# hugofloresgarcia/vampnet

Hardware: NVIDIA H100
Metric: codec tokens/sec (coarse 12 steps + c2f 24 steps generate, T=768, 44.1 kHz) (higher is better)
Workload: dtype bf16

## Files before the change

### vampnet_b200/csrc/api.cu

```cuda
#include <cuda_bf16.h>
#include <cudaTypedefs.h>

#include <cmath>
#include <cstdarg>
#include <cstdio>
#include <cstring>
#include <map>
#include <memory>
#include <string>
#include <tuple>
#include <vector>

#include "kernels.h"

namespace vnb {

static thread_local std::string g_err;
static thread_local std::string g_tmap_err;

static int fail(const char* fmt, ...) {
  char buf[1024];
  va_list ap;
  va_start(ap, fmt);
  vsnprintf(buf, sizeof(buf), fmt, ap);
  va_end(ap);
  g_err = buf;
  return 1;
}
#define CK(expr)                                                                                   \
  do {                                                                                             \
    cudaError_t _e = (expr);                                                                       \
    if (_e != cudaSuccess) return fail("%s failed: %s (%s:%d)", #expr, cudaGetErrorString(_e), __FILE__, __LINE__); \
  } while (0)

static PFN_cuTensorMapEncodeTiled_v12000 get_encode() {
  static PFN_cuTensorMapEncodeTiled_v12000 fn = nullptr;
  if (fn) return fn;
  void* p = nullptr;
  cudaDriverEntryPointQueryResult q;
  cudaError_t e = cudaGetDriverEntryPoint("cuTensorMapEncodeTiled", &p, cudaEnableDefault, &q);
  if (e != cudaSuccess || q != cudaDriverEntryPointSuccess || !p) {
    g_tmap_err = std::string("cudaGetDriverEntryPoint(cuTensorMapEncodeTiled) failed: ") + cudaGetErrorString(e);
    return nullptr;
  }
  fn = reinterpret_cast<PFN_cuTensorMapEncodeTiled_v12000>(p);
  return fn;
}
const char* tmap_error() { return g_tmap_err.c_str(); }

bool make_tmap_2d(CUtensorMap* tm, const void* base, uint64_t rows, uint64_t cols, uint32_t box_rows,
                  uint32_t box_cols) {
  auto enc = get_encode();
  if (!enc) return false;
  cuuint64_t dims[2] = {cols, rows};
  cuuint64_t strides[1] = {cols * 2};
  cuuint32_t box[2] = {box_cols, box_rows};
  cuuint32_t estr[2] = {1, 1};
  CUresult r = enc(tm, CU_TENSOR_MAP_DATA_TYPE_BFLOAT16, 2, const_cast<void*>(base), dims, strides, box, estr,
                   CU_TENSOR_MAP_INTERLEAVE_NONE, CU_TENSOR_MAP_SWIZZLE_128B, CU_TENSOR_MAP_L2_PROMOTION_L2_256B,
                   CU_TENSOR_MAP_FLOAT_OOB_FILL_NONE);
  if (r != CUDA_SUCCESS) {
    char b[256];
    snprintf(b, sizeof(b), "cuTensorMapEncodeTiled(2d rows=%llu cols=%llu box=%ux%u) -> %d", (unsigned long long)rows,
             (unsigned long long)cols, box_rows, box_cols, (int)r);
    g_tmap_err = b;
    return false;
  }
  return true;
}
bool make_tmap_3d(CUtensorMap* tm, const void* base, uint64_t batch, uint64_t rows, uint64_t cols,
                  uint64_t pitch_elems, uint32_t box_rows, uint32_t box_cols) {
  auto enc = get_encode();
  if (!enc) return false;
  cuuint64_t dims[3] = {cols, rows, batch};
  cuuint64_t strides[2] = {pitch_elems * 2, rows * pitch_elems * 2};
  cuuint32_t box[3] = {box_cols, box_rows, 1};
  cuuint32_t estr[3] = {1, 1, 1};
  CUresult r = enc(tm, CU_TENSOR_MAP_DATA_TYPE_BFLOAT16, 3, const_cast<void*>(base), dims, strides, box, estr,
                   CU_TENSOR_MAP_INTERLEAVE_NONE, CU_TENSOR_MAP_SWIZZLE_128B, CU_TENSOR_MAP_L2_PROMOTION_L2_256B,
                   CU_TENSOR_MAP_FLOAT_OOB_FILL_NONE);
  if (r != CUDA_SUCCESS) {
    char b[256];
    snprintf(b, sizeof(b), "cuTensorMapEncodeTiled(3d batch=%llu rows=%llu cols=%llu pitch=%llu box=%ux%u) -> %d",
             (unsigned long long)batch, (unsigned long long)rows, (unsigned long long)cols,
             (unsigned long long)pitch_elems, box_rows, box_cols, (int)r);
    g_tmap_err = b;
    return false;
  }
  return true;
}

static bool make_gemm_plan(GemmPlan* p, int epi, const void* A, const void* W, int M, int N, int K, void* out,
                           void* out2, const float* bias, int T, int Tpad, const float* ss_in, int ss_parts,
                           float inv_d, float eps, void* out_bf16, float* ss_out) {
  if (N % 256 != 0 || K % 64 != 0 || M < 1) {
    g_tmap_err = "gemm: need N % 256 == 0 and K % 64 == 0";
    return false;
  }
  GemmArgs& a = p->args;
  a.M = M; a.N = N; a.K = K; a.epi = epi; a.out = out; a.out2 = out2; a.bias = bias;
  a.T = T; a.Tpad = Tpad; a.d2 = epi == VNB_EPI_QKV ? (N / 3) * 2 : 0;
  if (ss_in != nullptr) { a.ss_in = ss_in; a.ss_parts = ss_parts; a.inv_d = inv_d; a.eps = eps; }
  a.out_bf16 = reinterpret_cast<__nv_bfloat16*>(out_bf16); a.ss_out = ss_out;
  return make_tmap_2d(&p->tmA, A, M, K, 128, 64) && make_tmap_2d(&p->tmB, W, N, K, 256, 64) &&
         make_tmap_2d(&p->tmBh, W, N, K, 128, 64);
}

bool make_attn_plan(AttnPlan* p, const void* qk, const void* vT, void* out, const float* rel, int sat, int B, int T,
                    int Tpad, int H) {
  const int d = H * 64;
  p->out = out; p->rel = rel; p->sat = sat; p->B = B; p->T = T; p->Tpad = Tpad; p->H = H;
  return make_tmap_3d(&p->tmQ, qk, B, T, 2 * d, 2 * d, 128, 64) && make_tmap_3d(&p->tmK, qk, B, T, 2 * d, 2 * d, 64, 64) &&
         make_tmap_3d(&p->tmVT, vT, B, d, Tpad, Tpad, 64, 64);
}

struct DevBuf {
  void* p = nullptr;
  size_t n = 0;
  ~DevBuf() { if (p) cudaFree(p); }
  cudaError_t alloc(size_t bytes, bool zero = false) {
    n = bytes;
    cudaError_t e = cudaMalloc(&p, bytes ? bytes : 1);
    if (e == cudaSuccess && zero) e = cudaMemset(p, 0, bytes);
    return e;
  }
  template <class T> T* as() const { return reinterpret_cast<T*>(p); }
};

struct Variant {
  int steps = 0;
  bool has_mask = false;
  bool top_p = false;
  int gemm_pair = 0;
  bool fused = false;
  bool adapted = false;
  bool ragged = false;
  bool mixed_steps = false;
  bool split = false;
  bool operator<(const Variant& o) const {
    return std::tie(steps, has_mask, top_p, gemm_pair, fused, adapted, ragged, mixed_steps, split) <
           std::tie(o.steps, o.has_mask, o.top_p, o.gemm_pair, o.fused, o.adapted, o.ragged, o.mixed_steps, o.split);
  }
};

struct Workspace {
  int B = 0, T = 0, Tpad = 0, M = 0;
  unsigned long long last_use = 0;
  DevBuf x, y, qk, vT, att, h, logits, zcur, zorig, tokens, conf, n0, dyn, rowgrp, z_in, mask_in, z_out, ssA, ssB, embA,
      partials;
  DevBuf grp_adapter, lora_u;
  DevBuf frames;
  DevBuf live;
  int embKp = 0;
  int ss_parts = 0;
  std::vector<GemmPlan> qkv, wo, up, down;
  GemmPlan cls, emb;
  GemmPlan cls_sample;
  bool can_fuse = false;
  AttnPlan attn;
  std::map<Variant, cudaGraphExec_t> graphs;
  std::map<Variant, unsigned long long> graph_kernels;
  ~Workspace() { for (auto& kv : graphs) cudaGraphExecDestroy(kv.second); }
};

}

namespace vnb {
enum { FAM_EMBED = 0, FAM_RMSNORM, FAM_GEMM_QKV, FAM_ATTN, FAM_GEMM_O, FAM_GEMM_UP, FAM_GEMM_DOWN, FAM_GEMM_CLS,
       FAM_SAMPLE, FAM_STATE, FAM_LORA_DOWN, FAM_COUNT };
static unsigned long long g_captures = 0;
static unsigned long long g_launches = 0;
void count_launch(unsigned long long n) { g_launches += n; }
struct Profiler {
  bool on = false;
  std::vector<cudaEvent_t> pool;
  std::vector<int> fam;
  size_t used = 0;
  ~Profiler() { for (auto e : pool) cudaEventDestroy(e); }
  void mark(int family, cudaStream_t st) {
    if (!on) return;
    if (used == pool.size()) {
      cudaEvent_t e;
      if (cudaEventCreate(&e) != cudaSuccess) { on = false; return; }
      pool.push_back(e);
      fam.push_back(-1);
    }
    fam[used] = family;
    cudaEventRecord(pool[used++], st);
// ... 1180 lines not shown
```

### vampnet_b200/csrc/common.cuh

```cuda
#pragma once
#include <cuda.h>
#include <cuda_bf16.h>
#include <cuda_runtime.h>
#include <stdint.h>
#include <stdio.h>

namespace vnb {

__device__ __forceinline__ uint32_t smem_u32(const void* p) {
  return static_cast<uint32_t>(__cvta_generic_to_shared(p));
}
__device__ __forceinline__ uint32_t lane_id() { return threadIdx.x & 31; }

__device__ __forceinline__ bool elect_one() {
  uint32_t pred = 0;
  asm volatile(
      "{\n\t.reg .pred P;\n\t.reg .b32 R;\n\t"
      "elect.sync R|P, 0xffffffff;\n\t"
      "selp.u32 %0, 1, 0, P;\n\t}"
      : "=r"(pred));
  return pred != 0;
}

__device__ __forceinline__ void mbar_init(uint64_t* bar, uint32_t count) {
  asm volatile("mbarrier.init.shared::cta.b64 [%0], %1;" ::"r"(smem_u32(bar)), "r"(count) : "memory");
}
__device__ __forceinline__ void mbar_fence_init() {
  asm volatile("fence.mbarrier_init.release.cluster;" ::: "memory");
}
__device__ __forceinline__ void mbar_expect_tx(uint64_t* bar, uint32_t bytes) {
  asm volatile("mbarrier.arrive.expect_tx.shared::cta.b64 _, [%0], %1;" ::"r"(smem_u32(bar)), "r"(bytes)
               : "memory");
}
__device__ __forceinline__ void mbar_arrive(uint64_t* bar) {
  asm volatile("mbarrier.arrive.shared::cta.b64 _, [%0];" ::"r"(smem_u32(bar)) : "memory");
}
__device__ __forceinline__ bool mbar_try_wait(uint64_t* bar, uint32_t parity) {
  uint32_t ok;
  asm volatile(
      "{\n\t.reg .pred P;\n\t"
      "mbarrier.try_wait.parity.shared::cta.b64 P, [%1], %2, %3;\n\t"
      "selp.u32 %0, 1, 0, P;\n\t}"
      : "=r"(ok)
      : "r"(smem_u32(bar)), "r"(parity), "r"(100000u)
      : "memory");
  return ok != 0;
}
__device__ __forceinline__ uint64_t global_timer_ns() {
  uint64_t t;
  asm volatile("mov.u64 %0, %%globaltimer;" : "=l"(t));
  return t;
}
#ifndef VNB_WAIT_TIMEOUT_NS
#define VNB_WAIT_TIMEOUT_NS 4000000000ull
#endif
__device__ __forceinline__ void mbar_wait(uint64_t* bar, uint32_t parity) {
  if (mbar_try_wait(bar, parity)) return;
  const uint64_t t0 = global_timer_ns();
  while (!mbar_try_wait(bar, parity))
    if (global_timer_ns() - t0 > VNB_WAIT_TIMEOUT_NS) __trap();
}

__device__ __forceinline__ void mbar_init_a(uint32_t bar, uint32_t count) {
  asm volatile("mbarrier.init.shared::cta.b64 [%0], %1;" ::"r"(bar), "r"(count) : "memory");
}
__device__ __forceinline__ void mbar_expect_tx_a(uint32_t bar, uint32_t bytes) {
  asm volatile("mbarrier.arrive.expect_tx.shared::cta.b64 _, [%0], %1;" ::"r"(bar), "r"(bytes) : "memory");
}
__device__ __forceinline__ void mbar_arrive_a(uint32_t bar) {
  asm volatile("mbarrier.arrive.shared::cta.b64 _, [%0];" ::"r"(bar) : "memory");
}
__device__ __forceinline__ bool mbar_try_wait_a(uint32_t bar, uint32_t parity) {
  uint32_t ok;
  asm volatile(
      "{\n\t.reg .pred P;\n\t"
      "mbarrier.try_wait.parity.shared::cta.b64 P, [%1], %2, %3;\n\t"
      "selp.u32 %0, 1, 0, P;\n\t}"
      : "=r"(ok)
      : "r"(bar), "r"(parity), "r"(100000u)
      : "memory");
  return ok != 0;
}
__device__ __forceinline__ void mbar_wait_a(uint32_t bar, uint32_t parity) {
  if (mbar_try_wait_a(bar, parity)) return;
  const uint64_t t0 = global_timer_ns();
  while (!mbar_try_wait_a(bar, parity))
    if (global_timer_ns() - t0 > VNB_WAIT_TIMEOUT_NS) __trap();
}

__device__ __forceinline__ void fence_proxy_async_smem() {
  asm volatile("fence.proxy.async.shared::cta;" ::: "memory");
}

__device__ __forceinline__ void tma_prefetch_desc(const CUtensorMap* m) {
  asm volatile("prefetch.tensormap [%0];" ::"l"(reinterpret_cast<uint64_t>(m)) : "memory");
}
__device__ __forceinline__ void tma_load_2d(void* dst, const CUtensorMap* m, uint64_t* bar, int c0, int c1) {
  asm volatile(
      "cp.async.bulk.tensor.2d.shared::cluster.global.mbarrier::complete_tx::bytes [%0], [%1, {%3, %4}], [%2];"
      ::"r"(smem_u32(dst)), "l"(reinterpret_cast<uint64_t>(m)), "r"(smem_u32(bar)), "r"(c0), "r"(c1)
      : "memory");
}
__device__ __forceinline__ void tma_load_3d(void* dst, const CUtensorMap* m, uint64_t* bar, int c0, int c1, int c2) {
  asm volatile(
      "cp.async.bulk.tensor.3d.shared::cluster.global.mbarrier::complete_tx::bytes [%0], [%1, {%3, %4, %5}], [%2];"
      ::"r"(smem_u32(dst)), "l"(reinterpret_cast<uint64_t>(m)), "r"(smem_u32(bar)), "r"(c0), "r"(c1), "r"(c2)
      : "memory");
}

__device__ __forceinline__ void tma_load_3d_a(uint32_t dst, const CUtensorMap* m, uint32_t bar, int c0, int c1, int c2) {
  asm volatile(
      "cp.async.bulk.tensor.3d.shared::cluster.global.mbarrier::complete_tx::bytes [%0], [%1, {%3, %4, %5}], [%2];"
      ::"r"(dst), "l"(reinterpret_cast<uint64_t>(m)), "r"(bar), "r"(c0), "r"(c1), "r"(c2)
      : "memory");
}

__device__ __forceinline__ void tma_store_2d(const CUtensorMap* m, const void* src, int c0, int c1) {
  asm volatile("cp.async.bulk.tensor.2d.global.shared::cta.bulk_group [%0, {%2, %3}], [%1];"
               ::"l"(reinterpret_cast<uint64_t>(m)), "r"(smem_u32(src)), "r"(c0), "r"(c1)
               : "memory");
}
__device__ __forceinline__ void bulk_commit() { asm volatile("cp.async.bulk.commit_group;" ::: "memory"); }
template <int N>
__device__ __forceinline__ void bulk_wait_read() {
  asm volatile("cp.async.bulk.wait_group.read %0;" ::"n"(N) : "memory");
}

__device__ __forceinline__ uint32_t cluster_ctarank() {
  uint32_t r;
  asm volatile("mov.u32 %0, %%cluster_ctarank;" : "=r"(r));
  return r;
}
__device__ __forceinline__ void cluster_sync_all() {
  asm volatile("barrier.cluster.arrive.release.aligned;\n\tbarrier.cluster.wait.acquire.aligned;" ::: "memory");
}
__device__ __forceinline__ uint32_t mapa_u32(uint32_t cta_addr, uint32_t rank) {
  uint32_t r;
  asm volatile("mapa.shared::cluster.u32 %0, %1, %2;" : "=r"(r) : "r"(cta_addr), "r"(rank));
  return r;
}
__device__ __forceinline__ void mbar_arrive_cluster(uint32_t cluster_addr) {
  asm volatile("mbarrier.arrive.release.cluster.shared::cluster.b64 _, [%0];" ::"r"(cluster_addr) : "memory");
}
__device__ __forceinline__ bool mbar_try_wait_cluster(uint64_t* bar, uint32_t parity) {
  uint32_t ok;
  asm volatile(
      "{\n\t.reg .pred P;\n\t"
      "mbarrier.try_wait.parity.acquire.cluster.shared::cta.b64 P, [%1], %2, %3;\n\t"
      "selp.u32 %0, 1, 0, P;\n\t}"
      : "=r"(ok)
      : "r"(smem_u32(bar)), "r"(parity), "r"(100000u)
      : "memory");
  return ok != 0;
}
__device__ __forceinline__ void mbar_wait_cluster(uint64_t* bar, uint32_t parity) {
  if (mbar_try_wait_cluster(bar, parity)) return;
  const uint64_t t0 = global_timer_ns();
  while (!mbar_try_wait_cluster(bar, parity))
    if (global_timer_ns() - t0 > VNB_WAIT_TIMEOUT_NS) __trap();
}
__device__ __forceinline__ void tma_load_2d_mc(void* dst, const CUtensorMap* m, uint64_t* bar, int c0, int c1,
                                               uint16_t cta_mask) {
  asm volatile(
      "cp.async.bulk.tensor.2d.shared::cluster.global.mbarrier::complete_tx::bytes.multicast::cluster"
      " [%0], [%1, {%3, %4}], [%2], %5;"
      ::"r"(smem_u32(dst)), "l"(reinterpret_cast<uint64_t>(m)), "r"(smem_u32(bar)), "r"(c0), "r"(c1), "h"(cta_mask)
      : "memory");
}

__device__ __forceinline__ uint32_t pack_bf16x2(float lo, float hi) {
  __nv_bfloat162 v = __floats2bfloat162_rn(lo, hi);
  return *reinterpret_cast<uint32_t*>(&v);
}
__device__ __forceinline__ float fast_exp2(float x) {
  float y;
  asm volatile("ex2.approx.ftz.f32 %0, %1;" : "=f"(y) : "f"(x));
  return y;
}
__device__ __forceinline__ float lds_f32(uint32_t addr) {
  float v;
  asm volatile("ld.shared.f32 %0, [%1];" : "=f"(v) : "r"(addr));
  return v;
}
__device__ __forceinline__ void sts_f32(uint32_t addr, float v) {
  asm volatile("st.shared.f32 [%0], %1;" ::"r"(addr), "f"(v) : "memory");
}
__device__ __forceinline__ void sts_u32(uint32_t addr, uint32_t v) {
  asm volatile("st.shared.b32 [%0], %1;" ::"r"(addr), "r"(v) : "memory");
}
__device__ __forceinline__ float4 lds_f4(uint32_t addr) {
  float4 v;
  asm volatile("ld.shared.v4.f32 {%0, %1, %2, %3}, [%4];" : "=f"(v.x), "=f"(v.y), "=f"(v.z), "=f"(v.w) : "r"(addr));
  return v;
}
__device__ __forceinline__ uint2 lds_u2(uint32_t addr) {
  uint2 v;
  asm volatile("ld.shared.v2.b32 {%0, %1}, [%2];" : "=r"(v.x), "=r"(v.y) : "r"(addr));
  return v;
}
__device__ __forceinline__ void sts_f4(uint32_t addr, float4 v) {
  asm volatile("st.shared.v4.f32 [%0], {%1, %2, %3, %4};" ::"r"(addr), "f"(v.x), "f"(v.y), "f"(v.z), "f"(v.w)
               : "memory");
}
__device__ __forceinline__ void sts_v4(uint32_t addr, uint32_t a, uint32_t b, uint32_t c, uint32_t d) {
  asm volatile("st.shared.v4.b32 [%0], {%1, %2, %3, %4};" ::"r"(addr), "r"(a), "r"(b), "r"(c), "r"(d) : "memory");
}
__device__ __forceinline__ float warp_max(float v) {
#pragma unroll
  for (int o = 16; o > 0; o >>= 1) v = fmaxf(v, __shfl_xor_sync(0xffffffffu, v, o));
  return v;
}
__device__ __forceinline__ float warp_sum(float v) {
#pragma unroll
  for (int o = 16; o > 0; o >>= 1) v += __shfl_xor_sync(0xffffffffu, v, o);
  return v;
}

__device__ __forceinline__ void philox4x32_10(uint32_t c0, uint32_t c1, uint32_t c2, uint32_t c3, uint32_t k0,
                                              uint32_t k1, uint32_t (&out)[4]) {
#pragma unroll
  for (int r = 0; r < 10; ++r) {
    const uint32_t hi0 = __umulhi(0xD2511F53u, c0), lo0 = 0xD2511F53u * c0;
    const uint32_t hi1 = __umulhi(0xCD9E8D57u, c2), lo1 = 0xCD9E8D57u * c2;
    const uint32_t n0 = hi1 ^ c1 ^ k0, n2 = hi0 ^ c3 ^ k1;
    c0 = n0; c1 = lo1; c2 = n2; c3 = lo0;
    k0 += 0x9E3779B9u;
    k1 += 0xBB67AE85u;
  }
  out[0] = c0; out[1] = c1; out[2] = c2; out[3] = c3;
}
__device__ __forceinline__ float u01(uint32_t x) { return (static_cast<float>(x >> 9) + 0.5f) * 1.1920928955078125e-07f; }

}
```

### vampnet_b200/csrc/gemm_wgmma.cu

```cuda
#include <stdlib.h>

#include "common.cuh"
#include "kernels.h"
#include "wgmma.cuh"

#ifndef VNB_GEMM_PAIR_DEFAULT
#define VNB_GEMM_PAIR_DEFAULT false
#endif

namespace vnb {

constexpr int BM = 128, BN = 256, BK = 64, STAGES = 4;
constexpr int A_BYTES = BM * BK * 2;
constexpr int B_BYTES = BN * BK * 2;
constexpr int STAGE_BYTES = A_BYTES + B_BYTES;
constexpr int SBIAS_BYTES = BN * 4;
constexpr int RING_BYTES = STAGES * STAGE_BYTES;
constexpr int ACC_PITCH = BN + 1;
static_assert(BM * ACC_PITCH * 4 <= RING_BYTES, "the accumulator tile overlays the ring");
static_assert(BM * ACC_PITCH * 4 + 4 * BM + 16 + 32 * BM <= RING_BYTES, "the adapted epilogue's row table follows it");
constexpr int GEMM_SMEM = RING_BYTES + SBIAS_BYTES + 1024  + 256 ;
static_assert(GEMM_SMEM <= 227 * 1024, "H100: at most 227 KiB of shared memory per block");
constexpr int GEMM_THREADS = 256 + 32;
template <int EPI> constexpr int gemm_epi_warps() { return (EPI == VNB_EPI_RESID || EPI == VNB_EPI_SAMPLE) ? 8 : 4; }
// ... 83 lines not shown
    const float rsr = __shfl_sync(0xffffffffu, rs, r);
    const uint32_t sp = quad + 4u * (r * ACC_PITCH + tc + c8);
    float x[8];
#pragma unroll
    for (int k = 0; k < 8; ++k) {
      x[k] = lds_f32(sp + 4u * k) * rsr;
      if constexpr (GEGLU) x[k] = x[k] * gelu_tanh(lds_f32(sp + 4u * (128 + k)) * rsr);
    }
    const int row = row_base + r;
    if (row < M) {
      uint4 w;
      w.x = pack_bf16x2(x[0], x[1]);
      w.y = pack_bf16x2(x[2], x[3]);
      w.z = pack_bf16x2(x[4], x[5]);
      w.w = pack_bf16x2(x[6], x[7]);
      *reinterpret_cast<uint4*>(out + static_cast<size_t>(row) * pitch + oc + c8) = w;
    }
  }
}

__device__ __forceinline__ void acc_ld_x32(uint32_t addr, uint32_t (&v)[32]) {
#pragma unroll
  for (int j = 0; j < 32; ++j) v[j] = __float_as_uint(lds_f32(addr + 4u * j));
}

template <int EPI>
__device__ __forceinline__ void lora_update(const GemmArgs& g, uint8_t* scratch, uint32_t acc_tile, int m0, int n0) {
  int uoff = 0, brow0 = n0;
  if constexpr (EPI == VNB_EPI_QKV) {
    const int d = g.N / 3;
    if (n0 >= d && n0 < 2 * d) return;
    if (n0 >= 2 * d) { uoff = 8; brow0 = n0 - d; }
  }
  const AdapterRefs& L = g.lora;
  const int t = static_cast<int>(threadIdx.x);
  int32_t* sid = reinterpret_cast<int32_t*>(scratch);
  uint32_t* smask = reinterpret_cast<uint32_t*>(scratch + 4 * BM);
  float4* su = reinterpret_cast<float4*>(scratch + 4 * BM + 16);
  constexpr int R = EPI == VNB_EPI_QKV ? 16 : 8;
  if (t < BM) {
    const int m = m0 + t;
    const int id = m < g.M ? L.grp_adapter[L.rowgrp[m / L.rows_per_grp].group] : -1;
    sid[t] = id;
    if (id >= 0) {
      su[2 * t] = __ldg(reinterpret_cast<const float4*>(L.u + static_cast<size_t>(m) * R + uoff));
      su[2 * t + 1] = __ldg(reinterpret_cast<const float4*>(L.u + static_cast<size_t>(m) * R + uoff + 4));
    }
    uint32_t bits = 0;
    for (int a = 0; a < VNB_MAX_ADAPTERS; ++a) bits |= __ballot_sync(0xffffffffu, id == a) ? (1u << a) : 0u;
    if ((t & 31) == 0) smask[t >> 5] = bits;
  }
  asm volatile("bar.sync 1, 256;" ::: "memory");
  const uint32_t present = smask[0] | smask[1] | smask[2] | smask[3];
  const int nb = EPI == VNB_EPI_QKV ? 2 * (g.N / 3) : g.N;
  const int c0 = t & 63, rq = t >> 6;
  for (int a = 0; a < VNB_MAX_ADAPTERS; ++a) {
    if (!((present >> a) & 1u)) continue;
    const float* bp = L.table[a].b[L.slot] + (static_cast<size_t>(L.layer) * nb + brow0 + c0) * 8;
    float4 b0[4], b1[4];
#pragma unroll
    for (int j = 0; j < 4; ++j) {
      b0[j] = __ldg(reinterpret_cast<const float4*>(bp + 64 * 8 * j));
      b1[j] = __ldg(reinterpret_cast<const float4*>(bp + 64 * 8 * j + 4));
    }
#pragma unroll 4
    for (int i = 0; i < BM / 4; ++i) {
      const int r = rq + 4 * i;
      if (sid[r] != a) continue;
      const float4 ua = su[2 * r], ub = su[2 * r + 1];
      const uint32_t row_addr = acc_tile + 4u * (r * ACC_PITCH + c0);
#pragma unroll
      for (int j = 0; j < 4; ++j) {
        float s = __fmul_rn(ua.x, b0[j].x);
        s = __fmaf_rn(ua.y, b0[j].y, s); s = __fmaf_rn(ua.z, b0[j].z, s); s = __fmaf_rn(ua.w, b0[j].w, s);
        s = __fmaf_rn(ub.x, b1[j].x, s); s = __fmaf_rn(ub.y, b1[j].y, s); s = __fmaf_rn(ub.z, b1[j].z, s);
        s = __fmaf_rn(ub.w, b1[j].w, s);
        const uint32_t addr = row_addr + 4u * (64 * j);
        sts_f32(addr, __fadd_rn(lds_f32(addr), s));
      }
    }
  }
}

template <int NS, typename Release>
__device__ __forceinline__ void gemm_mainloop(float (&acc)[128], uint8_t* ring, uint64_t* full_bar, int num_kb, int wg,
                                              int& stage, uint32_t& phase, Release&& release) {
#pragma unroll
  for (int i = 0; i < 128; ++i) acc[i] = 0.f;
  for (int kb = 0; kb < num_kb; ++kb) {
    mbar_wait(&full_bar[stage], phase);
    const uint32_t sa = smem_u32(ring + stage * STAGE_BYTES) + wg * (64 * 128);
    const uint32_t sb = smem_u32(ring + stage * STAGE_BYTES + A_BYTES);
    wgmma_fence();
#pragma unroll
    for (int k = 0; k < BK / 16; ++k)
      wgmma_ss_n256(acc, wgmma_desc_sw128(sa + k * 32), wgmma_desc_sw128(sb + k * 32), 1u);
    wgmma_commit();
    wgmma_wait<1>();
    wgmma_fence_regs(acc);
    if (kb > 0) release(stage == 0 ? NS - 1 : stage - 1);
    if (++stage == NS) { stage = 0; phase ^= 1; }
  }
  wgmma_wait<0>();
  wgmma_fence_regs(acc);
  if (num_kb > 0) release(stage == 0 ? NS - 1 : stage - 1);
}

template <int EPI, bool PAIR, bool ADAPT = false, bool SPLIT = false>
__global__ void __launch_bounds__(GEMM_THREADS, 1)
gemm_wgmma_kernel(const __grid_constant__ CUtensorMap tmA, const __grid_constant__ CUtensorMap tmB,
                  const GemmArgs g) {
  extern __shared__ uint8_t smem_raw[];
  uint8_t* smem = reinterpret_cast<uint8_t*>((reinterpret_cast<uintptr_t>(smem_raw) + 1023) & ~uintptr_t(1023));
  float* sbias_all = reinterpret_cast<float*>(smem + RING_BYTES);
  uint64_t* full_bar = reinterpret_cast<uint64_t*>(smem + RING_BYTES + SBIAS_BYTES);
  uint64_t* empty_bar = full_bar + STAGES;

  const int warp = threadIdx.x >> 5;
  const int lane = threadIdx.x & 31;
  const uint32_t rank = PAIR ? cluster_ctarank() : 0u;
  const int tile = PAIR ? static_cast<int>(blockIdx.x >> 1) : static_cast<int>(blockIdx.x);
  constexpr int TM = PAIR ? 2 * BM : BM;
  const int num_n = g.N / BN;
  const int num_kb = g.K / BK;
  const int m0 = (tile / num_n) * TM + static_cast<int>(rank) * BM;
  const int n0 = (tile % num_n) * BN;
  if (g.live != nullptr && (tile / num_n) * TM >= live_rows(g)) return;

  if (warp == 8 && lane == 0) {
    tma_prefetch_desc(&tmA);
    tma_prefetch_desc(&tmB);
    for (int s = 0; s < STAGES; ++s) {
      mbar_init(&full_bar[s], 1);
      mbar_init(&empty_bar[s], 8 * (PAIR ? 2 : 1));
    }
    mbar_fence_init();
  }
  if constexpr (PAIR) cluster_sync_all();
  else __syncthreads();

  if (warp == 8) {
    if (lane == 0) {
      int stage = 0;
      uint32_t phase = 0;
      for (int kb = 0; kb < num_kb; ++kb) {
        if constexpr (PAIR) mbar_wait_cluster(&empty_bar[stage], phase ^ 1);
        else mbar_wait(&empty_bar[stage], phase ^ 1);
        uint8_t* sa = smem + stage * STAGE_BYTES;
        uint8_t* sb = sa + A_BYTES;
        mbar_expect_tx(&full_bar[stage], STAGE_BYTES);
        tma_load_2d(sa, &tmA, &full_bar[stage], kb * BK, m0);
        if constexpr (PAIR)
          tma_load_2d_mc(sb + rank * (B_BYTES / 2), &tmB, &full_bar[stage], kb * BK, n0 + static_cast<int>(rank) * (BN / 2),
                         uint16_t(3));
        else
          tma_load_2d(sb, &tmB, &full_bar[stage], kb * BK, n0);
        if (++stage == STAGES) { stage = 0; phase ^= 1; }
      }
    }
    __syncwarp();
  } else {
    const int wg = warp >> 2;
    {
      float acc[128];
      const uint32_t peer_empty = PAIR ? mapa_u32(smem_u32(empty_bar), rank ^ 1u) : 0u;
      int stage = 0;
      uint32_t phase = 0;
      gemm_mainloop<STAGES>(acc, smem, full_bar, num_kb, wg, stage, phase, [&](int s) {
        if (lane == 0) {
          mbar_arrive(&empty_bar[s]);
          if constexpr (PAIR) mbar_arrive_cluster(peer_empty + 8u * s);
        }
      });
      asm volatile("bar.sync 1, 256;" ::: "memory");
      const uint32_t acc_tile = smem_u32(smem);
      const int r = wg * 64 + (warp & 3) * 16 + (lane >> 2);
      const uint32_t p0 = acc_tile + 4u * (r * ACC_PITCH + 2 * (lane & 3));
#pragma unroll
      for (int i = 0; i < 32; ++i) {
        sts_f32(p0 + 32u * i, acc[4 * i]);
        sts_f32(p0 + 32u * i + 4, acc[4 * i + 1]);
        sts_f32(p0 + 4u * (8 * ACC_PITCH) + 32u * i, acc[4 * i + 2]);
        sts_f32(p0 + 4u * (8 * ACC_PITCH) + 32u * i + 4, acc[4 * i + 3]);
      }
      asm volatile("bar.sync 1, 256;" ::: "memory");
// ... 302 lines not shown
#pragma unroll
          for (int h = 0; h < 2; ++h) {
            const float rsr = h ? rs1 : rs0;
            const uint32_t own = pack_bf16x2(acc[4 * i + 2 * h] * rsr, acc[4 * i + 2 * h + 1] * rsr);
            const uint32_t peer = __shfl_xor_sync(0xffffffffu, own, 4);
            sts_u32(stage_tile + stage_off<256>(c, (r + 8 * h) >> 1),
                    odd ? __byte_perm(peer, own, 0x7632) : __byte_perm(own, peer, 0x5410));
          }
        }
      }
      mbar_arrive(out_full);
    }
  } else {
    const int e = warp - 8;
    __nv_bfloat16* const out = reinterpret_cast<__nv_bfloat16*>(g.out);
    const int pitch = EPI == VNB_EPI_GEGLU ? g.N / 2 : g.d2;
    auto row_scales = [&](int tile) {
      if (tile < tiles) {
        const int m0 = (tile / num_n) * BM;
        for (int j = e * 32 + lane; j < BM; j += 32 * PERS_EPI_WARPS) srs[j] = row_scale(g, m0 + j);
      }
      mbar_arrive(out_free);
    };
    row_scales(blockIdx.x);
    uint32_t it = 0;
    for (int tile = blockIdx.x; tile < tiles; tile += gridDim.x, ++it) {
      const int m0 = (tile / num_n) * BM, n0 = (tile % num_n) * BN;
      mbar_wait(out_full, it & 1u);
      if constexpr (EPI == VNB_EPI_GEGLU) {
#pragma unroll 4
        for (int u = e; u < BM / 2; u += PERS_EPI_WARPS) {
          const int rr = 2 * u + (lane >> 4);
          const float4 v = lds_f4(stage_tile + stage_off<256>(rr, 4 * (lane & 15)));
          if (m0 + rr < g.M)
            *reinterpret_cast<float4*>(out + static_cast<size_t>(m0 + rr) * pitch + (n0 >> 1) + 8 * (lane & 15)) = v;
        }
      } else if (n0 < g.d2) {
#pragma unroll 4
        for (int rr = e; rr < BM; rr += PERS_EPI_WARPS) {
          const float4 v = lds_f4(stage_tile + stage_off<512>(rr, 4 * lane));
          if (m0 + rr < g.M)
            *reinterpret_cast<float4*>(out + static_cast<size_t>(m0 + rr) * pitch + n0 + 8 * lane) = v;
        }
      } else {
        const int d = g.N - g.d2;
        uint16_t* const vt = reinterpret_cast<uint16_t*>(g.out2) + static_cast<size_t>(n0 - g.d2) * g.Tpad;
        size_t off[4];
        bool ok[4];
        int bk[4];
        uint32_t keep[2] = {0xffffffffu, 0xffffffffu};
#pragma unroll
        for (int k = 0; k < 4; ++k) {
          const int m = m0 + 4 * lane + k;
          bk[k] = m / g.T;
          const int t = m - bk[k] * g.T;
          ok[k] = m < g.M;
          off[k] = static_cast<size_t>(bk[k]) * d * g.Tpad + t;
          if (ok[k] && g.frames != nullptr && t >= __ldg(g.frames + bk[k])) keep[k >> 1] &= (k & 1) ? 0xffffu : 0xffff0000u;
        }
        const bool wide = ok[3] && bk[3] == bk[0] && (off[0] & 3) == 0 && (g.Tpad & 3) == 0 &&
                          (reinterpret_cast<uintptr_t>(g.out2) & 7) == 0;
#pragma unroll 2
        for (int c = e; c < BN; c += PERS_EPI_WARPS) {
          uint2 v = lds_u2(stage_tile + stage_off<256>(c, 2 * lane));
          v.x &= keep[0];
          v.y &= keep[1];
          uint16_t* const o = vt + static_cast<size_t>(c) * g.Tpad;
          if (wide) {
            *reinterpret_cast<uint2*>(o + off[0]) = v;
          } else {
#pragma unroll
            for (int k = 0; k < 4; ++k) {
              const uint32_t w = k < 2 ? v.x : v.y;
              if (ok[k]) o[off[k]] = static_cast<uint16_t>((k & 1) ? (w >> 16) : w);
            }
          }
        }
      }
      row_scales(tile + gridDim.x);
    }
  }
}

static int g_gemm_pair = -1;
void set_gemm_pair(int on) { g_gemm_pair = on ? 1 : 0; }
static bool gemm_pair_enabled() {
  if (g_gemm_pair < 0) {
    const char* e = getenv("VNB_GEMM_PAIR");
    g_gemm_pair = e != nullptr ? (e[0] == '1') : (VNB_GEMM_PAIR_DEFAULT ? 1 : 0);
  }
  return g_gemm_pair == 1;
}
int get_gemm_pair() { return gemm_pair_enabled() ? 1 : 0; }

static int g_max_clusters[6][64];
template <int EPI>
static cudaError_t init_epi() {
  static PerDeviceOnce once;
  int dev;
  if (!once.need(&dev)) return cudaSuccess;
  cudaError_t e = cudaFuncSetAttribute(gemm_wgmma_kernel<EPI, false>, cudaFuncAttributeMaxDynamicSharedMemorySize, GEMM_SMEM);
  if (e != cudaSuccess) return e;
  e = cudaFuncSetAttribute(gemm_wgmma_kernel<EPI, true>, cudaFuncAttributeMaxDynamicSharedMemorySize, GEMM_SMEM);
  if (e != cudaSuccess) return e;
  if constexpr (EPI == VNB_EPI_QKV || EPI == VNB_EPI_RESID || EPI == VNB_EPI_GEGLU) {
    e = cudaFuncSetAttribute(gemm_wgmma_kernel<EPI, false, true>, cudaFuncAttributeMaxDynamicSharedMemorySize, GEMM_SMEM);
    if (e != cudaSuccess) return e;
    e = cudaFuncSetAttribute(gemm_wgmma_kernel<EPI, true, true>, cudaFuncAttributeMaxDynamicSharedMemorySize, GEMM_SMEM);
    if (e != cudaSuccess) return e;
  }
  if constexpr (EPI == VNB_EPI_GEGLU || EPI == VNB_EPI_QKV) {
    e = cudaFuncSetAttribute(gemm_persistent_kernel<EPI>, cudaFuncAttributeMaxDynamicSharedMemorySize, pers_smem<EPI>());
    if (e != cudaSuccess) return e;
  }
  if constexpr (EPI == VNB_EPI_SAMPLE) {
    e = cudaFuncSetAttribute(gemm_wgmma_kernel<EPI, false, false, true>, cudaFuncAttributeMaxDynamicSharedMemorySize,
                             GEMM_SMEM);
    if (e != cudaSuccess) return e;
    e = cudaFuncSetAttribute(gemm_wgmma_kernel<EPI, true, false, true>, cudaFuncAttributeMaxDynamicSharedMemorySize,
                             GEMM_SMEM);
    if (e != cudaSuccess) return e;
  }
  cudaLaunchConfig_t q = {};
  q.gridDim = dim3(2 * device_sm_count());
  q.blockDim = dim3(GEMM_THREADS);
  q.dynamicSmemBytes = GEMM_SMEM;
  cudaLaunchAttribute qa[1];
  qa[0].id = cudaLaunchAttributeClusterDimension;
  qa[0].val.clusterDim.x = 2; qa[0].val.clusterDim.y = 1; qa[0].val.clusterDim.z = 1;
  q.attrs = qa; q.numAttrs = 1;
  int n = 0;
  e = cudaOccupancyMaxActiveClusters(&n, gemm_wgmma_kernel<EPI, true>, &q);
  if (e != cudaSuccess || n <= 0) { (void)cudaGetLastError(); n = device_sm_count() / 2; }
  if (dev >= 0 && dev < 64) g_max_clusters[EPI][dev] = n;
  once.mark(dev);
  return cudaSuccess;
}
cudaError_t prepare_gemm() {
  cudaError_t e;
  if ((e = init_epi<VNB_EPI_BF16>()) != cudaSuccess) return e;
  if ((e = init_epi<VNB_EPI_QKV>()) != cudaSuccess) return e;
  if ((e = init_epi<VNB_EPI_RESID>()) != cudaSuccess) return e;
  if ((e = init_epi<VNB_EPI_GEGLU>()) != cudaSuccess) return e;
  if ((e = init_epi<VNB_EPI_BIAS_F32>()) != cudaSuccess) return e;
  return init_epi<VNB_EPI_SAMPLE>();
}

int get_gemm_max_clusters() {
  int dev = 0;
  cudaGetDevice(&dev);
  if (prepare_gemm() != cudaSuccess || dev < 0 || dev >= 64) return 0;
  return g_max_clusters[VNB_EPI_RESID][dev];
}

template <int EPI, bool ADAPT = false, bool SPLIT = false>
static cudaError_t launch_epi(const GemmPlan& p, const GemmArgs& g, cudaStream_t st) {
  cudaError_t e = init_epi<EPI>();
  if (e != cudaSuccess) return e;
  if (gemm_pair_enabled()) {
    const int clusters = ((g.M + 2 * BM - 1) / (2 * BM)) * (g.N / BN);
    cudaLaunchConfig_t cfg = {};
    cfg.gridDim = dim3(2 * clusters);
    cfg.blockDim = dim3(GEMM_THREADS);
    cfg.dynamicSmemBytes = GEMM_SMEM;
    cfg.stream = st;
    cudaLaunchAttribute attr[1];
    attr[0].id = cudaLaunchAttributeClusterDimension;
    attr[0].val.clusterDim.x = 2; attr[0].val.clusterDim.y = 1; attr[0].val.clusterDim.z = 1;
    cfg.attrs = attr; cfg.numAttrs = 1;
    return cudaLaunchKernelEx(&cfg, gemm_wgmma_kernel<EPI, true, ADAPT, SPLIT>, p.tmA, p.tmBh, g);
  }
  const int tiles = ((g.M + BM - 1) / BM) * (g.N / BN);
  if constexpr ((EPI == VNB_EPI_GEGLU || EPI == VNB_EPI_QKV) && !ADAPT) {
    const int grid = tiles < device_sm_count() ? tiles : device_sm_count();
    gemm_persistent_kernel<EPI><<<grid, PERS_THREADS, pers_smem<EPI>(), st>>>(p.tmA, p.tmB, g);
    return cudaGetLastError();
  }
  gemm_wgmma_kernel<EPI, false, ADAPT, SPLIT><<<tiles, GEMM_THREADS, GEMM_SMEM, st>>>(p.tmA, p.tmB, g);
  return cudaGetLastError();
}

cudaError_t launch_gemm(const GemmPlan& p, cudaStream_t st) {
  GemmArgs g = p.args;
  if (g.epi != VNB_EPI_QKV) g.frames = nullptr;
  if (g.lora.table != nullptr) {
    if (!g.lora.grp_adapter || !g.lora.rowgrp || !g.lora.u || g.lora.rows_per_grp < 1) return cudaErrorInvalidValue;
    switch (g.epi) {
      case VNB_EPI_QKV: return launch_epi<VNB_EPI_QKV, true>(p, g, st);
      case VNB_EPI_RESID: return launch_epi<VNB_EPI_RESID, true>(p, g, st);
      case VNB_EPI_GEGLU: return launch_epi<VNB_EPI_GEGLU, true>(p, g, st);
      default: return cudaErrorInvalidValue;
    }
  }
  switch (g.epi) {
    case VNB_EPI_BF16: return launch_epi<VNB_EPI_BF16>(p, g, st);
    case VNB_EPI_QKV: return launch_epi<VNB_EPI_QKV>(p, g, st);
    case VNB_EPI_RESID: return launch_epi<VNB_EPI_RESID>(p, g, st);
    case VNB_EPI_GEGLU: return launch_epi<VNB_EPI_GEGLU>(p, g, st);
    case VNB_EPI_BIAS_F32: return launch_epi<VNB_EPI_BIAS_F32>(p, g, st);
    case VNB_EPI_SAMPLE:
      if (!g.zcur || !g.dyn || !g.rowgrp || !g.partials || !g.bias || g.V % 128 != 0 || g.V > 1024) return cudaErrorInvalidValue;
      if (p.sample_split) {
        if (!g.out) return cudaErrorInvalidValue;
        return launch_epi<VNB_EPI_SAMPLE, false, true>(p, g, st);
      }
      return launch_epi<VNB_EPI_SAMPLE>(p, g, st);
    default: return cudaErrorInvalidValue;
  }
}

__global__ void gemm_ref_kernel(const __nv_bfloat16* A, const __nv_bfloat16* W, int M, int N, int K, float* out) {
  const int n = blockIdx.x * blockDim.x + threadIdx.x;
  const int m = blockIdx.y;
  if (n >= N || m >= M) return;
  float acc = 0.f;
  for (int k = 0; k < K; ++k)
    acc += __bfloat162float(A[static_cast<size_t>(m) * K + k]) * __bfloat162float(W[static_cast<size_t>(n) * K + k]);
  out[static_cast<size_t>(m) * N + n] = acc;
}
cudaError_t launch_gemm_ref(const void* A, const void* W, int M, int N, int K, float* out, cudaStream_t st) {
  dim3 grid((N + 127) / 128, M);
  gemm_ref_kernel<<<grid, 128, 0, st>>>(reinterpret_cast<const __nv_bfloat16*>(A),
                                        reinterpret_cast<const __nv_bfloat16*>(W), M, N, K, out);
  return cudaGetLastError();
}

}
```

### vampnet_b200/csrc/kernels.h

```cpp
#pragma once
#include <cuda.h>
#include <cuda_bf16.h>
#include <cuda_runtime.h>
#include <stdint.h>

#include <functional>
#include <vector>

#include "../../include/vampnet_b200.h"

namespace vnb {

struct PerDeviceOnce {
  unsigned long long done = 0;
  bool need(int* dev_out) {
    int dev = 0;
    cudaGetDevice(&dev);
    *dev_out = dev;
    return dev >= 64 || !((done >> dev) & 1ull);
  }
  void mark(int dev) { if (dev < 64) done |= 1ull << dev; }
};
inline int device_sm_count() {
  static int sms[64] = {0};
  int dev = 0;
  cudaGetDevice(&dev);
  if (dev >= 64) { int n = 0; cudaDeviceGetAttribute(&n, cudaDevAttrMultiProcessorCount, dev); return n; }
  if (!sms[dev]) cudaDeviceGetAttribute(&sms[dev], cudaDevAttrMultiProcessorCount, dev);
  return sms[dev];
}

void count_launch(unsigned long long n = 1);

inline size_t align256(size_t n) { return (n + 255) & ~(size_t)255; }
inline size_t carve(size_t& o, size_t bytes) {
  const size_t at = o;
  o = align256(o + bytes);
  return at;
}

enum TableKind { TABLE_FFT, TABLE_MEL_BANK, TABLE_BEAT, TABLE_PITCH_BASIS };
cudaError_t device_table(const std::vector<double>& key, const std::function<std::vector<char>()>& build,
                         const char** dev);

bool make_tmap_2d(CUtensorMap* tm, const void* base, uint64_t rows, uint64_t cols, uint32_t box_rows,
                  uint32_t box_cols);
bool make_tmap_3d(CUtensorMap* tm, const void* base, uint64_t batch, uint64_t rows, uint64_t cols,
                  uint64_t pitch_elems, uint32_t box_rows, uint32_t box_cols);
const char* tmap_error();
}
extern "C" int32_t vnb_set_error_cuda(const char* what, int32_t cuda_error);
namespace vnb {

struct SampleDyn;
struct RowGroup {
  int32_t group, first;
};

enum { LORA_QKV = 0, LORA_WO, LORA_W1, LORA_W2, LORA_SLOTS };
struct AdapterDev {
  const float* a[LORA_SLOTS];
  const float* b[LORA_SLOTS];
};
struct AdapterRefs {
  const AdapterDev* table = nullptr;
  const int32_t* grp_adapter = nullptr;
  const RowGroup* rowgrp = nullptr;
  int rows_per_grp = 1;
  int slot = 0, layer = 0;
  float* u = nullptr;
};
cudaError_t launch_lora_down(const void* y, int M, int K, const AdapterRefs& r, const int32_t* live, int T,
                             cudaStream_t st);

struct GemmArgs {
  int M, N, K;
  int epi;
  void* out;
  void* out2;
  const float* bias;
  int T, Tpad;
  int d2;
  __nv_bfloat16* out_bf16;
  float* ss_out;
  const float* ss_in;
  int ss_parts;
  float inv_d, eps;
  const int32_t* zcur;
  const SampleDyn* dyn;
  const RowGroup* rowgrp;
  float4* partials;
  int C, ncc, V, mask_token;
  AdapterRefs lora;
  const int32_t* frames;
  const int32_t* live;
};
struct GemmPlan {
  CUtensorMap tmA, tmB;
  CUtensorMap tmBh;
  bool sample_split = false;
  GemmArgs args{};
};
cudaError_t launch_gemm(const GemmPlan& p, cudaStream_t st);
cudaError_t prepare_gemm();
void set_gemm_pair(int on);
int get_gemm_pair();
int get_gemm_max_clusters();
cudaError_t launch_gemm_ref(const void* A, const void* W, int M, int N, int K, float* out, cudaStream_t st);

struct AttnPlan {
  CUtensorMap tmQ;
  CUtensorMap tmK;
  CUtensorMap tmVT;
  void* out = nullptr;
  const float* rel = nullptr;
  const int32_t* frames = nullptr;
  const int32_t* live = nullptr;
  int sat = 0, B = 0, T = 0, Tpad = 0, H = 0;
};
bool make_attn_plan(AttnPlan* p, const void* qk, const void* vT, void* out, const float* rel, int sat, int B, int T,
                    int Tpad, int H);
cudaError_t launch_attention(const AttnPlan& p, cudaStream_t st);

cudaError_t launch_embed_gather(const int32_t* codes_btc, const float* latents, const float* table, void* A, int M, int T,
                                int C, int V1, int K, int Kp, float* ss, int zero_from, int ss_parts,
                                const int32_t* live, cudaStream_t st);

cudaError_t launch_gen_init(const int64_t* z, const int32_t* mask, int32_t* zcur, int32_t* zorig, int32_t* n0,
                            const RowGroup* rowgrp, int n_groups, int B, int C, int T, int ncc, int mask_token,
                            cudaStream_t st);
cudaError_t launch_gen_finish(const int32_t* tokens, const int32_t* zorig, int64_t* out, int B, int C, int T, int ncc,
                              cudaStream_t st);

struct SampleDyn {
  float inv_temp, gamma, temp_eff;
  int do_sample, is_last, step;
  uint32_t seed_lo, seed_hi;
  float top_p;
};
struct SampleArgs {
  const float* logits;
  int32_t* zcur;
  const int32_t* zorig;
  int32_t* tokens;
  float* conf;
  const int32_t* n0;
  const RowGroup* rowgrp;
  int B, T, C, ncc, V, mask_token;
  const int32_t* live = nullptr;
};
cudaError_t launch_sample_step_dev(const SampleArgs& a, const SampleDyn* dyn_dev, cudaStream_t st, bool use_top_p);
cudaError_t launch_sample_combine_dev(const SampleArgs& a, const void* partials, const SampleDyn* dyn_dev, cudaStream_t st);
cudaError_t launch_remask_dev(const SampleArgs& a, const SampleDyn* dyn_dev, cudaStream_t st);
cudaError_t launch_sample_split_dev(const SampleArgs& a, const void* partials, const SampleDyn* dyn_dev, cudaStream_t st);

struct FftTables {
  const float2* twiddle;
  const float* window;
};
cudaError_t fft_tables(int n_fft, FftTables* out);
struct MelBank {
  const float* w;
  const int32_t* off;
  const int32_t* lo;
};
cudaError_t mel_filterbank(int sr, int n_fft, int n_mels, double fmin, double fmax, MelBank* out);

enum class SpecMode { ONSET_DB, MEL_MAG };
constexpr int ONSET_NFFT = 2048, ONSET_NMELS = 128;
cudaError_t launch_spectrogram(SpecMode mode, const float* samples, int rows, int N, int hop, int n_fft,
                               const FftTables& fft, const MelBank& bank, int n_mels, float* out, cudaStream_t st);

struct OnsetGeometry {
  int pre_max = 0, post_max = 0, pre_avg = 0, post_avg = 0, wait = 0, pad = 0;
};
OnsetGeometry onset_geometry(int sr, int hop);
struct OnsetTables {
  FftTables fft;
  MelBank bank;
  OnsetGeometry g;
  float delta;
};
// ... 73 lines not shown
```

Before: 290,600.

## Add persistent warp-specialized residual GEMM with ping-pong consumer warpgroups

Adds a persistent residual-epilogue GEMM kernel with a dedicated TMA producer warp, register reallocation via setmaxnreg, and, for K up to 1280, two consumer warpgroups that ping-pong over 64-row tiles using named barriers. One group's epilogue (residual add, bf16 copy, sum-of-squares) overlaps the other group's mainloop. The epilogue now stages accumulators through a small per-warp shared buffer instead of the full tile. This adds a second tensor map and more complex barrier and phase bookkeeping, which risks ordering bugs.

```diff
diff --git a/vampnet_b200/csrc/api.cu b/vampnet_b200/csrc/api.cu
--- a/vampnet_b200/csrc/api.cu
+++ b/vampnet_b200/csrc/api.cu
@@ -103,7 +103,7 @@
   if (ss_in != nullptr) { a.ss_in = ss_in; a.ss_parts = ss_parts; a.inv_d = inv_d; a.eps = eps; }
   a.out_bf16 = reinterpret_cast<__nv_bfloat16*>(out_bf16); a.ss_out = ss_out;
   return make_tmap_2d(&p->tmA, A, M, K, 128, 64) && make_tmap_2d(&p->tmB, W, N, K, 256, 64) &&
-         make_tmap_2d(&p->tmBh, W, N, K, 128, 64);
+         make_tmap_2d(&p->tmBh, W, N, K, 128, 64) && (epi != VNB_EPI_RESID || make_tmap_2d(&p->tmA64, A, M, K, 64, 64));
 }
 
 bool make_attn_plan(AttnPlan* p, const void* qk, const void* vT, void* out, const float* rel, int sat, int B, int T,
diff --git a/vampnet_b200/csrc/common.cuh b/vampnet_b200/csrc/common.cuh
--- a/vampnet_b200/csrc/common.cuh
+++ b/vampnet_b200/csrc/common.cuh
@@ -88,6 +88,17 @@
     if (global_timer_ns() - t0 > VNB_WAIT_TIMEOUT_NS) __trap();
 }
 
+template <int N>
+__device__ __forceinline__ void setmaxnreg_dec() { asm volatile("setmaxnreg.dec.sync.aligned.u32 %0;" ::"n"(N)); }
+template <int N>
+__device__ __forceinline__ void setmaxnreg_inc() { asm volatile("setmaxnreg.inc.sync.aligned.u32 %0;" ::"n"(N)); }
+__device__ __forceinline__ void named_bar_sync(int id, int threads) {
+  asm volatile("bar.sync %0, %1;" ::"r"(id), "r"(threads) : "memory");
+}
+__device__ __forceinline__ void named_bar_arrive(int id, int threads) {
+  asm volatile("bar.arrive %0, %1;" ::"r"(id), "r"(threads) : "memory");
+}
+
 __device__ __forceinline__ void fence_proxy_async_smem() {
   asm volatile("fence.proxy.async.shared::cta;" ::: "memory");
 }
@@ -197,6 +208,9 @@
   uint2 v;
   asm volatile("ld.shared.v2.b32 {%0, %1}, [%2];" : "=r"(v.x), "=r"(v.y) : "r"(addr));
   return v;
+}
+__device__ __forceinline__ void sts_f2(uint32_t addr, float x, float y) {
+  asm volatile("st.shared.v2.f32 [%0], {%1, %2};" ::"r"(addr), "f"(x), "f"(y) : "memory");
 }
 __device__ __forceinline__ void sts_f4(uint32_t addr, float4 v) {
   asm volatile("st.shared.v4.f32 [%0], {%1, %2, %3, %4};" ::"r"(addr), "f"(v.x), "f"(v.y), "f"(v.z), "f"(v.w)
diff --git a/vampnet_b200/csrc/gemm_wgmma.cu b/vampnet_b200/csrc/gemm_wgmma.cu
--- a/vampnet_b200/csrc/gemm_wgmma.cu
+++ b/vampnet_b200/csrc/gemm_wgmma.cu
@@ -189,15 +189,19 @@
   }
 }
 
-template <int NS, typename Release>
+struct NoHook {
+  __device__ void operator()() const {}
+};
+template <int NS, int SB = STAGE_BYTES, int AB = A_BYTES, typename Release, typename Issued = NoHook>
 __device__ __forceinline__ void gemm_mainloop(float (&acc)[128], uint8_t* ring, uint64_t* full_bar, int num_kb, int wg,
-                                              int& stage, uint32_t& phase, Release&& release) {
+                                              int& stage, uint32_t& phase, Release&& release,
+                                              Issued&& issued = Issued()) {
 #pragma unroll
   for (int i = 0; i < 128; ++i) acc[i] = 0.f;
   for (int kb = 0; kb < num_kb; ++kb) {
     mbar_wait(&full_bar[stage], phase);
-    const uint32_t sa = smem_u32(ring + stage * STAGE_BYTES) + wg * (64 * 128);
-    const uint32_t sb = smem_u32(ring + stage * STAGE_BYTES + A_BYTES);
+    const uint32_t sa = smem_u32(ring + stage * SB) + wg * (64 * 128);
+    const uint32_t sb = smem_u32(ring + stage * SB + AB);
     wgmma_fence();
 #pragma unroll
     for (int k = 0; k < BK / 16; ++k)
@@ -208,6 +212,7 @@
     if (kb > 0) release(stage == 0 ? NS - 1 : stage - 1);
     if (++stage == NS) { stage = 0; phase ^= 1; }
   }
+  issued();
   wgmma_wait<0>();
   wgmma_fence_regs(acc);
   if (num_kb > 0) release(stage == 0 ? NS - 1 : stage - 1);
@@ -676,6 +681,157 @@
   }
 }
 
+constexpr int PP_THREADS = 384;
+constexpr int PP_MAX_K = 1280;
+constexpr int PP_RING = 5 * (64 * BK * 2 + B_BYTES);
+constexpr int PP_XPITCH = 40, PP_XBYTES = 16 * PP_XPITCH * 4;
+constexpr int PP_SMEM = PP_RING + 128  + 8 * PP_XBYTES + 1024 ;
+static_assert(4 * STAGE_BYTES <= PP_RING, "the 128-row ring fits");
+static_assert(PP_SMEM <= 227 * 1024, "H100: at most 227 KiB of shared memory per block");
+static_assert(2 * 5 * 8 <= 128, "the barriers fit their slot");
+static_assert(128 * 40 + 256 * 232 <= 384 * 168, "setmaxnreg: the register split fits the launch's 168 per thread");
+
+template <int TM>
+__global__ void __launch_bounds__(PP_THREADS, 1)
+gemm_resid_kernel(const __grid_constant__ CUtensorMap tmA, const __grid_constant__ CUtensorMap tmB,
+                  const GemmArgs g) {
+  constexpr bool PING = TM == 64;
+  constexpr int NS = PING ? 5 : 4;
+  constexpr int ABYTES = TM * BK * 2;
+  constexpr int SBYTES = ABYTES + B_BYTES;
+  static_assert(NS * SBYTES <= PP_RING, "the ring fits its space");
+  extern __shared__ uint8_t smem_raw[];
+  uint8_t* smem = reinterpret_cast<uint8_t*>((reinterpret_cast<uintptr_t>(smem_raw) + 1023) & ~uintptr_t(1023));
+  uint64_t* full_bar = reinterpret_cast<uint64_t*>(smem + PP_RING);
+  uint64_t* empty_bar = full_bar + NS;
+
+  const int warp = threadIdx.x >> 5;
+  const int lane = threadIdx.x & 31;
+  const int num_n = g.N / BN;
+  const int num_kb = g.K / BK;
+  const int tiles = ((live_rows(g) + TM - 1) / TM) * num_n;
+  const int first = static_cast<int>(blockIdx.x), stride = static_cast<int>(gridDim.x);
+  const int mine = tiles > first ? (tiles - first + stride - 1) / stride : 0;
+
+  if (threadIdx.x == 0) {
+    tma_prefetch_desc(&tmA);
+    tma_prefetch_desc(&tmB);
+    for (int s = 0; s < NS; ++s) {
+      mbar_init(&full_bar[s], 1);
+      mbar_init(&empty_bar[s], PING ? 4 : 8);
+    }
+    mbar_fence_init();
+  }
+  __syncthreads();
+
+  if (warp >= 8) {
+    setmaxnreg_dec<40>();
+    if (warp == 8 && lane == 0) {
+      int stage = 0;
+      uint32_t phase = 0;
+      for (int j = 0; j < mine; ++j) {
+        const int tile = first + j * stride;
+        const int m0 = (tile / num_n) * TM, n0 = (tile % num_n) * BN;
+        for (int kb = 0; kb < num_kb; ++kb) {
+          mbar_wait(&empty_bar[stage], phase ^ 1);
+          uint8_t* sa = smem + stage * SBYTES;
+          mbar_expect_tx(&full_bar[stage], SBYTES);
+          tma_load_2d(sa, &tmA, &full_bar[stage], kb * BK, m0);
+          tma_load_2d(sa + ABYTES, &tmB, &full_bar[stage], kb * BK, n0);
+          if (++stage == NS) { stage = 0; phase ^= 1; }
+        }
+      }
+    }
+    return;
+  }
+  setmaxnreg_inc<232>();
+  const int wg = warp >> 2;
+  if (PING && wg == 1 && mine > 0) named_bar_arrive(1, 256);
+  float* const out = reinterpret_cast<float*>(g.out);
+  const bool fused = g.out_bf16 != nullptr;
+  const uint32_t xb = smem_u32(smem + PP_RING + 128) + warp * PP_XBYTES;
+  const int cq = 2 * (lane & 3);
+  for (int j = PING ? wg : 0; j < mine; j += PING ? 2 : 1) {
+    const int tile = first + j * stride;
+    const int m0 = (tile / num_n) * TM + (PING ? 0 : wg * 64), n0 = (tile % num_n) * BN;
+    const int kb0 = j * num_kb;
+    int stage = kb0 % NS;
+    uint32_t phase = (kb0 / NS) & 1u;
+    float acc[128];
+    if (PING) named_bar_sync(1 + wg, 256);
+    gemm_mainloop<NS, SBYTES, ABYTES>(
+        acc, smem, full_bar, num_kb, PING ? 0 : wg, stage, phase,
+        [&](int s) { if (lane == 0) mbar_arrive(&empty_bar[s]); },
+        [&] { if (PING && j + 1 < mine) named_bar_arrive(2 - wg, 256); });
+
+    const int wrow = m0 + (warp & 3) * 16 + (lane >> 3);
+    const int c4 = (lane & 7) * 4;
+    const size_t step = static_cast<size_t>(4) * g.N;
+    float* const obase = out + static_cast<size_t>(wrow) * g.N + n0 + c4;
+    float rs[4];
+    bool ok[4];
+#pragma unroll
+    for (int it = 0; it < 4; ++it) {
+      rs[it] = row_scale(g, wrow + 4 * it);
+      ok[it] = wrow + 4 * it < g.M;
+    }
+    auto load = [&](int c, float4 (&v)[4]) {
+#pragma unroll
+      for (int it = 0; it < 4; ++it)
+        v[it] = ok[it] ? __ldcg(reinterpret_cast<const float4*>(obase + it * step + 32 * c)) : make_float4(0.f, 0.f, 0.f, 0.f);
+    };
+    float ssacc[2][4] = {};
+    float4 nxt[4];
+    load(0, nxt);
+#pragma unroll
+    for (int c = 0; c < BN / 32; ++c) {
+      float4 res[4];
+#pragma unroll
+      for (int it = 0; it < 4; ++it) res[it] = nxt[it];
+      if (c + 1 < BN / 32) load(c + 1, nxt);
+#pragma unroll
+      for (int k = 0; k < 4; ++k) {
+        const int i = 4 * c + k;
+        sts_f2(xb + 4u * ((lane >> 2) * PP_XPITCH + 8 * k + cq), acc[4 * i], acc[4 * i + 1]);
+        sts_f2(xb + 4u * (((lane >> 2) + 8) * PP_XPITCH + 8 * k + cq), acc[4 * i + 2], acc[4 * i + 3]);
+      }
+      __syncwarp();
+#pragma unroll
+      for (int it = 0; it < 4; ++it) {
+        float4 a = lds_f4(xb + 4u * ((it * 4 + (lane >> 3)) * PP_XPITCH + c4));
+        a = make_float4(__fmul_rn(a.x, rs[it]), __fmul_rn(a.y, rs[it]), __fmul_rn(a.z, rs[it]), __fmul_rn(a.w, rs[it]));
+        a.x = __fadd_rn(a.x, res[it].x); a.y = __fadd_rn(a.y, res[it].y);
+        a.z = __fadd_rn(a.z, res[it].z); a.w = __fadd_rn(a.w, res[it].w);
+        if (ok[it]) {
+          *reinterpret_cast<float4*>(obase + it * step + 32 * c) = a;
+          if (fused) {
+            uint2 w;
+            w.x = pack_bf16x2(a.x, a.y);
+            w.y = pack_bf16x2(a.z, a.w);
+            *reinterpret_cast<uint2*>(g.out_bf16 + static_cast<size_t>(wrow + 4 * it) * g.N + n0 + 32 * c + c4) = w;
+            ssacc[c & 1][it] = __fadd_rn(ssacc[c & 1][it], sumsq4(a.x, a.y, a.z, a.w));
+          }
+        }
+      }
+      __syncwarp();
+    }
+    if (fused) {
+#pragma unroll
+      for (int h = 0; h < 2; ++h) {
+#pragma unroll
+        for (int it = 0; it < 4; ++it) {
+          float v = ssacc[h][it];
+          v += __shfl_xor_sync(0xffffffffu, v, 1);
+          v += __shfl_xor_sync(0xffffffffu, v, 2);
+          v += __shfl_xor_sync(0xffffffffu, v, 4);
+          const int rr = wrow + 4 * it;
+          if ((lane & 7) == 0 && rr < g.M) g.ss_out[static_cast<size_t>((n0 / BN) * 2 + h) * g.M + rr] = v;
+        }
+      }
+    }
+  }
+}
+
 static int g_gemm_pair = -1;
 void set_gemm_pair(int on) { g_gemm_pair = on ? 1 : 0; }
 static bool gemm_pair_enabled() {
@@ -705,6 +861,12 @@
   }
   if constexpr (EPI == VNB_EPI_GEGLU || EPI == VNB_EPI_QKV) {
     e = cudaFuncSetAttribute(gemm_persistent_kernel<EPI>, cudaFuncAttributeMaxDynamicSharedMemorySize, pers_smem<EPI>());
+    if (e != cudaSuccess) return e;
+  }
+  if constexpr (EPI == VNB_EPI_RESID) {
+    e = cudaFuncSetAttribute(gemm_resid_kernel<64>, cudaFuncAttributeMaxDynamicSharedMemorySize, PP_SMEM);
+    if (e != cudaSuccess) return e;
+    e = cudaFuncSetAttribute(gemm_resid_kernel<128>, cudaFuncAttributeMaxDynamicSharedMemorySize, PP_SMEM);
     if (e != cudaSuccess) return e;
   }
   if constexpr (EPI == VNB_EPI_SAMPLE) {
@@ -770,6 +932,17 @@
     gemm_persistent_kernel<EPI><<<grid, PERS_THREADS, pers_smem<EPI>(), st>>>(p.tmA, p.tmB, g);
     return cudaGetLastError();
   }
+  if constexpr (EPI == VNB_EPI_RESID && !ADAPT) {
+    if (g.K <= PP_MAX_K) {
+      const int pp_tiles = ((g.M + 63) / 64) * (g.N / BN);
+      const int grid = pp_tiles < device_sm_count() ? pp_tiles : device_sm_count();
+      gemm_resid_kernel<64><<<grid, PP_THREADS, PP_SMEM, st>>>(p.tmA64, p.tmB, g);
+    } else {
+      const int grid = tiles < device_sm_count() ? tiles : device_sm_count();
+      gemm_resid_kernel<128><<<grid, PP_THREADS, PP_SMEM, st>>>(p.tmA, p.tmB, g);
+    }
+    return cudaGetLastError();
+  }
   gemm_wgmma_kernel<EPI, false, ADAPT, SPLIT><<<tiles, GEMM_THREADS, GEMM_SMEM, st>>>(p.tmA, p.tmB, g);
   return cudaGetLastError();
 }
diff --git a/vampnet_b200/csrc/kernels.h b/vampnet_b200/csrc/kernels.h
--- a/vampnet_b200/csrc/kernels.h
+++ b/vampnet_b200/csrc/kernels.h
@@ -98,6 +98,7 @@
 struct GemmPlan {
   CUtensorMap tmA, tmB;
   CUtensorMap tmBh;
+  CUtensorMap tmA64;
   bool sample_split = false;
   GemmArgs args{};
 };
```

Result: faster. 293,600, median of 6 (+1.0%).
